# bcsefercik/markerless-robot-camera-calibration

Measured on AMD Instinct MI355X. Metric: point-cloud frames/sec at 200k pts/frame, higher is better.
Workload: dtype f32

## Files before the change

### include/sv_hip.h

```cpp
#ifndef SV_HIP_H
#define SV_HIP_H

#include <stddef.h>
#include <stdint.h>

#ifdef __cplusplus
extern "C" {
#endif

#define SV_OK 0
#define SV_ERR_INVALID (-1)
#define SV_ERR_WORKSPACE (-2)
#define SV_ERR_HIP (-3)
#define SV_ERR_RANGE (-4)
#define SV_ERR_UNSUPPORTED (-5)

#define SV_ACT_NONE 0
#define SV_ACT_RELU 1
#define SV_ACT_LEAKY_RELU 2

#define SV_POOL_MAX 0
#define SV_POOL_AVG 1

#define SV_REDUCE_MEAN 0
// ... 269 lines not shown
                     int max_n, int64_t* out, sv_stream_t stream);
#define SV_PN_MAX_LAYERS 4
int sv_pointnet_sa(const float* xyz, const float* points, const float* new_xyz, const int64_t* group_idx, int B, int N,
                   int D, int S, int nsample, const float* params, const int* widths, int L, float* out,
                   sv_stream_t stream);
#define SV_PN_MAX_SCALES 4
int sv_pointnet_sa_msg(const float* xyz, const float* points, const float* new_xyz, int B, int N, int D, int S, int R,
                       const int* nsamples, const int64_t* const* group_idx, const float* const* params,
                       const int* widths, const int* nlayers, float* out, sv_stream_t stream);

#define SV_GROUP_SSG 0
#define SV_GROUP_MSG 1
int sv_group_rows(const float* xyz, const float* points, const float* new_xyz, const int64_t* idx, int B, int N, int D,
                  int S, int nsample, int order, int ld, float* out, sv_stream_t stream);
size_t sv_index_transpose_workspace_bytes(int B, int64_t M, int N);
int sv_index_transpose(const void* idx, int idx_bytes, int B, int64_t M, int N, void* workspace, size_t workspace_bytes,
                       int32_t* offsets, int32_t* pos, sv_stream_t stream);
int sv_gather_transpose(const int32_t* offsets, const int32_t* pos, const float* w, const float* rows, int64_t ld_rows,
                        int col0, int C, int per_row, int64_t T, float* out, int64_t ld_out, sv_stream_t stream);
int sv_group_max(const float* rows, int64_t ld, int64_t G, int nsample, int C, float* out, int32_t* arg,
                 sv_stream_t stream);
int sv_group_max_backward(const float* dpooled, const int32_t* arg, int64_t G, int nsample, int C, float* drows,
                          sv_stream_t stream);
int sv_three_nn(const float* xyz1, const float* xyz2, int B, int N, int S, int32_t* idx, float* w, sv_stream_t stream);
int sv_three_nn_gather(const float* points2, const int32_t* idx, const float* w, int B, int N, int S, int C, float* out,
                       sv_stream_t stream);

size_t sv_cluster_workspace_bytes(int64_t n);
int sv_single_linkage_roots(const void* xyz, int elem_bytes, int64_t ld, const int32_t* idx, int64_t n, double dist,
                            void* workspace, size_t workspace_bytes, int32_t* root, int32_t* best, sv_stream_t stream);
int sv_select_equal(const void* v, int elem_bytes, int64_t n, int64_t value, const int32_t* value_dev, int64_t* out,
                    int64_t* count, sv_stream_t stream);

#ifdef __cplusplus
}
#endif
#endif
```

### markerless-robot-camera-calibration_amd/_lib.py

```python
import ctypes
import os
import threading
from ctypes import c_char_p, c_double, c_float, c_int, c_int64, c_size_t, c_void_p

import torch

_HERE = os.path.dirname(os.path.abspath(__file__))
ABI_VERSION = 4
LIB_PATH = os.environ.get("SVHIP_LIB") or os.path.join(_HERE, "libsvhip.so")

SV_ACT_NONE, SV_ACT_RELU, SV_ACT_LEAKY_RELU = 0, 1, 2
SV_POOL_MAX, SV_POOL_AVG = 0, 1
SV_REDUCE_MEAN, SV_REDUCE_FIRST = 0, 1
SV_TILE_ROWS = 128
SV_ERR_UNSUPPORTED = -5
SV_PN_MAX_LAYERS = 4
SV_PN_MAX_SCALES = 4
SV_BQ_MAX_RADII = 4
SV_GROUP_SSG, SV_GROUP_MSG = 0, 1
SV_LOSS_POSE, SV_LOSS_SHAPE_MATCH, SV_LOSS_POSE_MATCH, SV_LOSS_KP_POSE_MATCH = 0, 1, 2, 3
SV_AUG_STRIDE, SV_AUG_ELASTIC0, SV_AUG_ELASTIC1 = 40, 0, 7
SV_AUG_E_ON, SV_AUG_E_OFFSET, SV_AUG_E_BX, SV_AUG_E_BY, SV_AUG_E_BZ, SV_AUG_E_GRAN, SV_AUG_E_MAG = range(7)
SV_AUG_NOISE_ON, SV_AUG_NOISE_SIGMA, SV_AUG_NOISE_CLIP, SV_AUG_TRANSFORM_ON, SV_AUG_ROT, SV_AUG_TRANSLATION = 14, 15, 16, 17, 18, 27
SV_AUG_FLIP_SIGN, SV_AUG_GRAVITY_ON, SV_AUG_GRAVITY_ANGLE, SV_AUG_GRAVITY_COS, SV_AUG_GRAVITY_SIN = 30, 31, 32, 33, 34
SV_ORIGIN_NONE, SV_ORIGIN_CENTER, SV_ORIGIN_BASE = 0, 1, 2
SV_COORD_BIAS = 1 << 17
SV_COORD_BITS = 18
SV_MAX_BATCH = 1024
SV_FRAME_MAX_LEVELS, SV_FRAME_MAX_CUTS, SV_FRAME_RECORD = 8, 4, 16
SV_FRAME_K3, SV_FRAME_DOWN, SV_FRAME_UP, SV_FRAME_SPLIT = 1, 2, 4, 8
SV_FIELD_F32, SV_FIELD_F64 = 7, 8
SV_UNPACK_BIGENDIAN, SV_UNPACK_KEEP_NONFINITE = 1, 2
SV_DEPTH_U16, SV_DEPTH_F32 = 4, 7
SV_RGBD_ALIGNED, SV_RGBD_NEAREST, SV_RGBD_BGR = 1, 2, 4
SV_CONV_SEL_PLAN, SV_CONV_SEL_TILE_ORDER, SV_CONV_SEL_VEC_A, SV_CONV_SEL_BUF_OK, SV_CONV_SEL_ACC_INIT, SV_CONV_SEL_W_ALIGNED = (
    1, 2, 4, 8, 16, 32)
SV_FRAME_REC_HASH, SV_FRAME_REC_K3, SV_FRAME_REC_DOWN, SV_FRAME_REC_UP, SV_FRAME_REC_SPLIT = 1, 2, 3, 4, 5


class SvHipError(RuntimeError):
    pass


_P = c_void_p
SIGNATURES = {
    "sv_last_error": (c_char_p, []),
    "sv_abi_version": (c_int, []),
    "sv_voxelize_workspace_bytes": (c_size_t, [c_int64]),
    "sv_voxelize": (c_int, [_P, c_int, c_int64, _P, c_size_t, _P, _P, _P, _P, _P, _P, _P]),
    "sv_voxel_reduce": (c_int, [_P, c_int, _P, _P, c_int64, c_int, _P, _P]),
    "sv_hash_build": (c_int, [_P, c_int64, _P, _P, c_int64, _P]),
    "sv_stride_map_workspace_bytes": (c_size_t, [c_int64]),
    "sv_stride_map": (c_int, [_P, c_int64, c_int, _P, c_size_t, _P, _P, _P, _P, _P, _P]),
    "sv_kernel_map_k3": (c_int, [_P, c_int64, c_int, c_int, _P, _P, c_int64, _P, c_int64, _P, _P]),
    "sv_kernel_map_down": (c_int, [_P, _P, c_int64, c_int, c_int64, _P, c_int64, _P, _P]),
    "sv_kernel_map_up": (c_int, [_P, _P, c_int64, c_int, _P, c_int64, _P, _P]),
    "sv_plan_workspace_bytes": (c_size_t, [c_int64]),
    "sv_plan_build": (c_int, [_P, c_int64, _P, c_int, c_int64, c_int64, _P, c_size_t, _P, _P, _P, _P, c_int64, _P]),
    "sv_conv_fwd": (
        c_int,
        [_P, c_int64, c_int64, c_int, _P, c_int, c_int, _P, _P, _P, _P, c_int64, c_int64, _P, _P, _P, c_int64, c_int,
         c_float, _P, c_int64, _P],
    ),
    "sv_conv_fwd_acc": (
        c_int,
        [_P, c_int64, c_int64, c_int, _P, c_int, c_int, _P, _P, _P, _P, c_int64, c_int64, _P, c_int64, _P, _P, _P, c_int64, c_int,
         c_float, _P, c_int64, _P],
    ),
    "sv_pack_weights_bf16": (c_int, [_P, c_int, c_int, c_int, _P, _P]),
    "sv_conv_fwd_bf16": (
# ... 64 lines not shown
    "sv_pose_match_loss": (c_int, [_P, _P, c_int64, c_int, _P, _P, _P, _P, _P, _P, c_int, _P, c_size_t, _P, _P, _P, _P, _P]),
    "sv_elastic_field_workspace_bytes": (c_size_t, [_P, c_int]),
    "sv_elastic_field": (c_int, [_P, _P, c_int, _P, c_size_t, _P, _P]),
    "sv_augment_points_workspace_bytes": (c_size_t, [c_int64, c_int]),
    "sv_augment_points": (c_int, [_P, c_int, _P, c_int64, c_int, _P, _P, c_int64, _P, _P, c_size_t, _P, _P, _P]),
    "sv_quantise_points": (c_int, [_P, _P, c_int64, c_int, _P, c_int, c_double, _P, _P, _P, _P]),
    "sv_ee_mask": (c_int, [_P, c_int, _P, c_int64, c_int, _P, _P, _P, _P, _P]),
    "sv_key_points": (c_int, [_P, c_int, _P, c_int64, c_int, _P, _P, c_int, c_double, c_int64, _P, _P, _P, _P]),
    "sv_line_topk_workspace_bytes": (c_size_t, [c_int64]),
    "sv_line_topk": (c_int, [_P, c_int, _P, c_int64, c_int, _P, _P, _P, _P, c_int, c_double, _P, c_size_t, _P, _P, _P, _P]),
    "sv_radius_labels": (c_int, [_P, c_int, _P, c_int64, c_int, _P, c_int, c_double, c_int64, _P, _P]),
    "sv_seg_criterion_workspace_bytes": (c_size_t, [c_int64, c_int, c_int]),
    "sv_seg_criterion": (c_int, [_P, c_int64, c_int, c_int64, _P, c_int64, _P, c_int, _P, c_size_t, _P, _P, _P, _P, _P, _P]),
    "sv_segment_topk_workspace_bytes": (c_size_t, [c_int64, c_int, c_int]),
    "sv_segment_topk": (c_int, [_P, c_int64, c_int64, _P, c_int, c_int, _P, c_size_t, _P, _P]),
    "sv_fps": (c_int, [_P, c_int, c_int, c_int, _P, _P, _P]),
    "sv_three_nn_interpolate": (c_int, [_P, _P, _P, c_int, c_int, c_int, c_int, _P, _P]),
    "sv_cluster_workspace_bytes": (c_size_t, [c_int64]),
    "sv_single_linkage_roots": (c_int, [_P, c_int, c_int64, _P, c_int64, c_double, _P, c_size_t, _P, _P, _P]),
    "sv_select_equal": (c_int, [_P, c_int, c_int64, c_int64, _P, _P, _P, _P]),
    "sv_ball_query": (c_int, [_P, _P, c_int, c_int, c_int, c_double, c_int, _P, _P]),
    "sv_fps_segmented": (c_int, [_P, _P, _P, _P, c_int, c_int, _P, _P]),
    "sv_pointnet_sa": (c_int, [_P, _P, _P, _P, c_int, c_int, c_int, c_int, c_int, _P, _P, c_int, _P, _P]),
    "sv_ball_query_multi": (c_int, [_P, _P, c_int, c_int, c_int, c_int, _P, _P, _P, _P]),
    "sv_pointnet_sa_msg": (c_int, [_P, _P, _P, c_int, c_int, c_int, c_int, c_int, _P, _P, _P, _P, _P, _P, _P]),
    "sv_group_rows": (c_int, [_P, _P, _P, _P, c_int, c_int, c_int, c_int, c_int, c_int, c_int, _P, _P]),
    "sv_index_transpose_workspace_bytes": (c_size_t, [c_int, c_int64, c_int]),
    "sv_index_transpose": (c_int, [_P, c_int, c_int, c_int64, c_int, _P, c_size_t, _P, _P, _P]),
    "sv_gather_transpose": (c_int, [_P, _P, _P, _P, c_int64, c_int, c_int, c_int, c_int64, _P, c_int64, _P]),
    "sv_group_max": (c_int, [_P, c_int64, c_int64, c_int, c_int, _P, _P, _P]),
    "sv_group_max_backward": (c_int, [_P, _P, c_int64, c_int, c_int, _P, _P]),
    "sv_three_nn": (c_int, [_P, _P, c_int, c_int, c_int, _P, _P, _P]),
    "sv_three_nn_gather": (c_int, [_P, _P, _P, c_int, c_int, c_int, c_int, _P, _P]),
}

_lib = None


def load():
    global _lib
    if _lib is not None:
        return _lib
    if not os.path.exists(LIB_PATH):
        raise SvHipError(
            f"{LIB_PATH} not found: build it with `python -c 'import __graft_entry__ as g; g.build()'` "
            "(or `make -C markerless-robot-camera-calibration_amd/csrc`). There is no CPU fallback."
        )
    lib = ctypes.CDLL(LIB_PATH)
    lib.sv_abi_version.restype = c_int
    if lib.sv_abi_version() != ABI_VERSION:
        raise SvHipError(f"{LIB_PATH} has C-ABI version {lib.sv_abi_version()}, this package binds version {ABI_VERSION}: "
                         "rebuild it (`python -c 'import __graft_entry__ as g; g.build()'`)")
    for name, (res, args) in SIGNATURES.items():
        fn = getattr(lib, name)
        fn.restype = res
        fn.argtypes = args
    _lib = lib
    return lib


def _check(rc, name):
    if rc != 0:
        msg = _lib.sv_last_error().decode("utf-8", "replace")
        raise SvHipError(f"{name} failed with status {rc}: {msg}")


# ... 62 lines not shown
```

### markerless-robot-camera-calibration_amd/model/robotnet.py

```python
import torch
import torch.nn as nn
import torch.nn.functional as F

from .. import MinkowskiEngine as ME
from .. import nn as svnn
from .._lib import SV_ACT_LEAKY_RELU, SV_ACT_RELU
from ..utils import config
from ._select import pose_backbone


def _linear_fused(linear, x, act=0, slope=0.01):
    w3 = linear.weight.detach().t().contiguous().unsqueeze(0)
    bias = linear.bias.detach() if linear.bias is not None else None
    return svnn.conv_forward(x.contiguous(), w3, None, x.shape[0], None, bias, None, act, slope)


class _PoseHeadMixin:
    def _init_head(self, feat_channels, out_channels, avg_pool):
        cfg = config.Config()
        self.global_pool = ME.MinkowskiGlobalAvgPooling() if avg_pool else ME.MinkowskiGlobalMaxPooling()
        self.final_bn = ME.MinkowskiBatchNorm(out_channels)
        self.output_layer = nn.Sequential(ME.MinkowskiBatchNorm(feat_channels), self.relu)
        self.use_joint_angles = bool(cfg.STRUCTURE.use_joint_angles)
        self.pose_regression_input_size = feat_channels + (9 if self.use_joint_angles else 0)
        self.pose_regression = nn.Sequential(
            nn.Linear(self.pose_regression_input_size, 2048),
            nn.LeakyReLU(),
            nn.Linear(2048, out_channels),
        )

    def _regress(self, feats, joint_angles):
        if self.training:
            return self._regress_train(feats, joint_angles)
        scale, shift = self.output_layer[0].folded()
        feats = feats.new(svnn.affine_act(feats.F, scale, shift, act=SV_ACT_RELU))
        pooled = self.global_pool(feats).features
        if self.use_joint_angles:
            pooled = torch.cat((pooled, joint_angles.to(pooled)), dim=1)
        h = _linear_fused(self.pose_regression[0], pooled, SV_ACT_LEAKY_RELU, self.pose_regression[1].negative_slope)
        out = _linear_fused(self.pose_regression[2], h)
        out[:, 7:] = torch.sigmoid(out[:, 7:])
        if not self.training:
            out[:, 3:7] = F.normalize(out[:, 3:7], p=2, dim=1)
        return out


    def _regress_train(self, feats, joint_angles):
        feats = self.relu(self.output_layer[0](feats))
        pooled = self.global_pool(feats).features
        if self.use_joint_angles:
            pooled = torch.cat((pooled, joint_angles.to(pooled)), dim=1)
        h = svnn.linear_train(self.pose_regression[0], pooled, SV_ACT_LEAKY_RELU, self.pose_regression[1].negative_slope)
        out = svnn.linear_train(self.pose_regression[2], h)
        return torch.cat((out[:, :7], torch.sigmoid(out[:, 7:])), dim=1)


def make_robotnet(backbone=None):
    UNet = pose_backbone(backbone, "ROTATION")

    class RobotNet(UNet, _PoseHeadMixin):
        name = "robotnet"

        def __init__(self, in_channels, out_channels, D=3):
            UNet.__init__(self, in_channels, out_channels, D)
            self.leaky_relu = ME.MinkowskiLeakyReLU(inplace=False)
            self._init_head(self.PLANES[-1] * self.BLOCK.expansion, out_channels, avg_pool=False)

        def forward(self, x):
            joint_angles = None
            if isinstance(x, tuple):
                x, joint_angles = x
            return self._regress(self.forward_except_final(x), joint_angles)

    return RobotNet


def make_robotnet_encode(backbone=None):
    UNet = pose_backbone(backbone, "TRANSLATION")

    class RobotNetEncode(UNet, _PoseHeadMixin):
        name = "robotnet"

        def __init__(self, in_channels, out_channels, D=3):
            UNet.__init__(self, in_channels, out_channels, D)
            cfg = config.Config()
            self.leaky_relu = nn.LeakyReLU()
            self._init_head(self.PLANES[3] * self.BLOCK.expansion, out_channels, avg_pool=True)
            self.quantization_size = cfg()["DATA"].get("quantization_size", 1 / cfg.DATA.scale)
            self.voxelize_position = cfg()["DATA"].get("voxelize_position", False)

        def forward(self, x):
            joint_angles = None
            if isinstance(x, tuple):
                x, joint_angles = x
            out = self.conv0p1s1.forward_fused(x, bn=self.bn0, act=SV_ACT_RELU)
            for i in range(1, 5):
                conv, bn, block = self._down_names(i)
                out = getattr(self, conv).forward_fused(out, bn=getattr(self, bn), act=SV_ACT_RELU)
                out = getattr(self, block)(out)
            out = self._regress(out, joint_angles)
            if not self.training and self.voxelize_position:
                out[:, :3] *= self.quantization_size
            return out

    return RobotNetEncode


RobotNet = make_robotnet()
```

### markerless-robot-camera-calibration_amd/model/robotnet_segmentation.py

```python
import torch.nn as nn

from .. import MinkowskiEngine as ME
from .._lib import SV_ACT_LEAKY_RELU
from ..utils import config
from ._select import pose_backbone, segmentation_backbone

EPS = 1e-6


def _classification_head(UNet, default_classes, class_name):
    class _Head(UNet):
        name = "robotnet"

        def __init__(self, in_channels, out_channels=256, D=3, num_classes=None):
            UNet.__init__(self, in_channels, out_channels, D)
            if num_classes is None:
                num_classes = default_classes()
            self.leaky_relu = ME.MinkowskiLeakyReLU()
            self.regression = nn.Sequential(
                ME.MinkowskiOps.MinkowskiLinear(256, 1024),
                ME.MinkowskiLeakyReLU(),
                ME.MinkowskiOps.MinkowskiLinear(1024, num_classes),
            )
            self.sigm = ME.MinkowskiSigmoid()

        def forward(self, x):
            if isinstance(x, tuple):
                x, _joint_angles = x
            slope = self.leaky_relu.negative_slope
            out = UNet.forward(self, x, final_act=SV_ACT_LEAKY_RELU, final_slope=slope)
            out = self.regression[0].forward_fused(out, act=SV_ACT_LEAKY_RELU,
                                                   slope=self.regression[1].negative_slope)
            return self.regression[2].forward_fused(out)

    _Head.__name__ = _Head.__qualname__ = class_name
    return _Head


def make_robotnet_segmentation(backbone=None):
    return _classification_head(segmentation_backbone(backbone), lambda: config.Config().DATA.classes,
                                "RobotNetSegmentation")


def make_robotnet_vote(backbone=None):
    return _classification_head(pose_backbone(backbone, "ROTATION"),
                                lambda: 2 if config.Config().DATA.data_type == "ee_seg" else 4, "RobotNetVote")


RobotNetSegmentation = make_robotnet_segmentation()
```

### markerless-robot-camera-calibration_amd/nn.py

```python
import math
from ctypes import c_float, c_int, c_int64, c_size_t

import numpy as np
import torch
import torch.nn as nn

from . import _lib, profiling
from ._lib import SV_ACT_LEAKY_RELU, SV_ACT_NONE, SV_ACT_RELU, call, ptr, stream_ptr
from .sparse import SparseTensor, SplitPlan

KERNEL_OFFSET_PERMUTATION = None

import os as _os


def _parse_split_rules(text):
    rules = []
    for part in text.split(";"):
        if part.strip():
            rows, _, cuts = part.partition(":")
            cuts = tuple(int(v) for v in cuts.split(",") if v)
            rules.append((int(rows), cuts[0] if len(cuts) == 1 else cuts))
    return sorted(rules, key=lambda r: -r[0])


SPLIT_RULES = _parse_split_rules(_os.environ.get("MRCC_SPLIT_RULES", "20000:9,18"))
SPLIT_MIN_CHANNELS = int(_os.environ.get("MRCC_SPLIT_MIN_CHANNELS", "128"))


SPLIT_RULES_ONE_FRAME = _parse_split_rules(_os.environ.get("MRCC_SPLIT_RULES_ONE_FRAME", "50000:9,18"))


def split_points_for(rows):
    for min_rows, cuts in SPLIT_RULES:
        if rows >= min_rows:
            return cuts
    return None


def conv_forward(feats, weight3, plan, V_out, scale=None, shift=None, residual=None, act=SV_ACT_NONE, slope=0.01,
                 out=None, weight_bf16=None):
    K, Cin, Cout = weight3.shape
    if feats.shape[1] != Cin:
        raise ValueError(f"input has {feats.shape[1]} channels, kernel expects {Cin}")
    if feats.stride(1) != 1:
        feats = feats.contiguous()
    if out is None:
        out = torch.empty((V_out, Cout), dtype=torch.float32, device=feats.device)
    if isinstance(plan, SplitPlan):
        return _conv_forward_split(feats, weight3, plan, V_out, scale, shift, residual, act, slope, out, weight_bf16)
    return _conv_forward_one(feats, weight3, plan, V_out, scale, shift, residual, act, slope, out, None, wp=weight_bf16)


def pack_weights_bf16(weight3):
    K, Cin, Cout = weight3.shape
    w = weight3.detach().float().contiguous()
    wp = torch.empty(K * Cin * Cout, dtype=torch.bfloat16, device=w.device)
    call("sv_pack_weights_bf16", ptr(w), c_int(K), c_int(Cin), c_int(Cout), ptr(wp), stream_ptr())
    return wp


def _conv_forward_split(feats, weight3, plan, V_out, scale, shift, residual, act, slope, out, weight_bf16=None):
    K, Cin, Cout = weight3.shape
    timer = profiling.TIMER
    t0 = None
    if timer is not None:
        kname = profiling.conv_kernel_config(Cout, plan.Vpad, Cin, plan.parts[-1][1] - plan.parts[-1][0])
        if timer.want(kname):
            t0 = timer.start()
    if weight_bf16 is None and not weight3.is_contiguous():
        weight3 = weight3.contiguous()
    acc = None
    for i, (k0, k1, sub) in enumerate(plan.parts):
        w = weight3[k0:k1]
        wp = weight_bf16[k0 * Cin * Cout:k1 * Cin * Cout] if weight_bf16 is not None else None
        if i == len(plan.parts) - 1:
            _conv_forward_one(feats, w, sub, V_out, scale, shift, residual, act, slope, out, acc, timed=False, wp=wp)
        else:
            nxt = torch.empty((V_out, Cout), dtype=torch.float32, device=feats.device)
            _conv_forward_one(feats, w, sub, V_out, None, None, None, SV_ACT_NONE, slope, nxt, acc, timed=False, wp=wp)
            acc = nxt
    if t0 is not None:
        timer.stop(t0, _lib.conv_last_instance()[0], K, Cin, Cout, V_out, plan.pairs_device(), level=plan.out_stride,
                   passes=len(plan.parts))
# ... 613 lines not shown
```

### markerless-robot-camera-calibration_amd/profiling.py

```python
import math

import torch

from . import _lib

TIMER = None
INSTANCE_LOG = None
TRAIN_LOG = None


def conv_kernel_config(Cout, Vpad, Cin, K=1):
    flags = _lib.SV_CONV_SEL_BUF_OK | _lib.SV_CONV_SEL_W_ALIGNED
    if K > 1:
        flags |= _lib.SV_CONV_SEL_PLAN | _lib.SV_CONV_SEL_TILE_ORDER
    if Cin % 4 == 0:
        flags |= _lib.SV_CONV_SEL_VEC_A
    return _lib.conv_instance(K, Cin, Cout, Vpad, flags).partition("|")[0]


class KernelTimer:
    def __init__(self, capacity=0):
        self.records = []
        self.enabled = True
        self.only = None
        self._pool = [torch.cuda.Event(enable_timing=True) for _ in range(capacity)]
        self._next = 0
        self._first_of_frame = False

    def _event(self):
        if self._next < len(self._pool):
            e = self._pool[self._next]
            self._next += 1
            return e
        return torch.cuda.Event(enable_timing=True)

    def want(self, kernel):
        return self.enabled and (self.only is None or kernel in self.only)

    def start(self):
        e = self._event()
        e.record()
        return e

    def stop(self, start_evt, kernel, K, Cin, Cout, V_out, pairs_dev, level=None, passes=1):
        e = self._event()
        e.record()
        self.records.append((kernel, K, Cin, Cout, V_out, pairs_dev, start_evt, e, self._first_of_frame, level, passes))
        self._first_of_frame = False

    def frame_boundary(self):
        self._first_of_frame = True

    def clear(self):
        self.records = []

    @staticmethod
    def layer_key(kernel, K, Cin, Cout, V_out, level=None):
        where = f"s{level}" if level is not None else f"~2^{int(round(math.log2(max(V_out, 1))))}"
        return (kernel, K, Cin, Cout, where)

    def summarize(self, by_layer=False):
        out = {}
        for kernel, K, Cin, Cout, V_out, pairs_dev, s, e, first, level, passes in self.records:
            if first:
                continue
            P = int(pairs_dev.item()) if pairs_dev is not None else V_out
            ms = s.elapsed_time(e)
            key = self.layer_key(kernel, K, Cin, Cout, V_out, level) if by_layer else kernel
            d = out.setdefault(key, {"launches": 0, "ms": 0.0, "flops": 0.0, "bytes": 0.0, "rows": 0.0, "kernel_launches": 0})
            d["rows"] += V_out
            d["launches"] += 1
            d["kernel_launches"] += passes
            d["ms"] += ms
            d["flops"] += 2.0 * P * Cin * Cout
            d["bytes"] += P * (4.0 * Cin + 8) + 4.0 * V_out * Cout + 4.0 * K * Cin * Cout
        return out


def pass_gflop(fn):
    global TIMER
# ... 8 lines not shown
```

Measured before the change: 74.65.

## Compile eval network into an op program executed by one native call

Adds a net executor that compiles the RobotNet/segmentation forward into a flat array of op records (conv, bf16 conv, column copy, affine, pool, event wait/record). A single C entry point then launches them all in sequence. Activations live in one preallocated arena with precomputed offsets, and concatenations become column copies into that arena. The aim is to remove per-layer Python dispatch, tensor allocation and ctypes overhead in inference. It adds a large compile and layout-check layer and falls back to layer-by-layer execution for unrecognised modules.

```diff
diff --git a/include/sv_hip.h b/include/sv_hip.h
--- a/include/sv_hip.h
+++ b/include/sv_hip.h
@@ -325,6 +325,41 @@
 int sv_select_equal(const void* v, int elem_bytes, int64_t n, int64_t value, const int32_t* value_dev, int64_t* out,
                     int64_t* count, sv_stream_t stream);
 
+#define SV_NET_NOP 0
+#define SV_NET_CONV 1
+#define SV_NET_CONV_BF16 2
+#define SV_NET_COPY_COLS 3
+#define SV_NET_AFFINE 4
+#define SV_NET_POOL 5
+#define SV_NET_WAIT_EVENT 6
+#define SV_NET_RECORD_EVENT 7
+#define SV_NET_NAME_BYTES 128
+typedef struct sv_net_op {
+  int32_t kind, Cin, K, Cout, act;
+  float slope;
+  int32_t B, mode;
+  const void* in;
+  int64_t V_in, in_ld;
+  const void* W;
+  const int32_t* perm;
+  const int32_t* nbr_s;
+  const uint32_t* submask;
+  const int32_t* tile_order;
+  int64_t V_out, Vpad;
+  const float* acc_init;
+  int64_t acc_ld;
+  const float* scale;
+  const float* shift;
+  const float* residual;
+  int64_t res_ld;
+  void* out;
+  int64_t out_ld;
+  void* event;
+  char* name_host;
+} sv_net_op;
+int sv_net_op_layout(int64_t* out_host, int capacity);
+int sv_net_forward(const sv_net_op* ops, int n, int* failed_index, sv_stream_t stream);
+
 #ifdef __cplusplus
 }
 #endif
diff --git a/markerless-robot-camera-calibration_amd/_lib.py b/markerless-robot-camera-calibration_amd/_lib.py
--- a/markerless-robot-camera-calibration_amd/_lib.py
+++ b/markerless-robot-camera-calibration_amd/_lib.py
@@ -36,6 +36,9 @@
 SV_CONV_SEL_PLAN, SV_CONV_SEL_TILE_ORDER, SV_CONV_SEL_VEC_A, SV_CONV_SEL_BUF_OK, SV_CONV_SEL_ACC_INIT, SV_CONV_SEL_W_ALIGNED = (
     1, 2, 4, 8, 16, 32)
 SV_FRAME_REC_HASH, SV_FRAME_REC_K3, SV_FRAME_REC_DOWN, SV_FRAME_REC_UP, SV_FRAME_REC_SPLIT = 1, 2, 3, 4, 5
+(SV_NET_NOP, SV_NET_CONV, SV_NET_CONV_BF16, SV_NET_COPY_COLS, SV_NET_AFFINE, SV_NET_POOL, SV_NET_WAIT_EVENT,
+ SV_NET_RECORD_EVENT) = range(8)
+SV_NET_NAME_BYTES = 128
 
 
 class SvHipError(RuntimeError):
@@ -166,6 +169,8 @@
     "sv_group_max_backward": (c_int, [_P, _P, c_int64, c_int, c_int, _P, _P]),
     "sv_three_nn": (c_int, [_P, _P, c_int, c_int, c_int, _P, _P, _P]),
     "sv_three_nn_gather": (c_int, [_P, _P, _P, c_int, c_int, c_int, c_int, _P, _P]),
+    "sv_net_op_layout": (c_int, [_P, c_int]),
+    "sv_net_forward": (c_int, [_P, c_int, _P, _P]),
 }
 
 _lib = None
diff --git a/markerless-robot-camera-calibration_amd/csrc/sv_net.hip b/markerless-robot-camera-calibration_amd/csrc/sv_net.hip
--- /dev/null
+++ b/markerless-robot-camera-calibration_amd/csrc/sv_net.hip
@@ -0,0 +1,110 @@
+#include <stddef.h>
+#include <string.h>
+
+#include "sv_common.h"
+
+namespace sv {
+
+template <typename T>
+__global__ __launch_bounds__(256) void copy_cols_kernel(const T* __restrict__ in, int64_t in_ld, T* __restrict__ out, int64_t out_ld,
+                                                        int64_t rows, int cols) {
+  const int64_t total = rows * (int64_t)cols;
+  for (int64_t i = (int64_t)blockIdx.x * blockDim.x + threadIdx.x; i < total; i += (int64_t)gridDim.x * blockDim.x) {
+    const int64_t r = i / cols;
+    const int c = (int)(i - r * cols);
+    out[r * out_ld + c] = in[r * in_ld + c];
+  }
+}
+
+static int copy_cols(const sv_net_op& op, hipStream_t stream) {
+  const float* in = (const float*)op.in;
+  float* out = (float*)op.out;
+  const int cols = op.Cout;
+  const int64_t rows = op.V_out;
+  SV_CHECK_ARG(cols > 0 && rows >= 0 && op.in_ld >= cols && op.out_ld >= cols, "bad column count / row strides");
+  if (rows == 0) return SV_OK;
+  SV_CHECK_ARG(in && out, "null pointer");
+  const bool vec = cols % 4 == 0 && op.in_ld % 4 == 0 && op.out_ld % 4 == 0 && (((uintptr_t)in | (uintptr_t)out) & 15) == 0;
+  const int64_t total = rows * (int64_t)(vec ? cols / 4 : cols);
+  int64_t blocks = (total + 255) / 256;
+  if (blocks > 65536) blocks = 65536;
+  if (vec)
+    copy_cols_kernel<float4><<<dim3((unsigned)blocks), dim3(256), 0, stream>>>((const float4*)in, op.in_ld / 4, (float4*)out, op.out_ld / 4,
+                                                                              rows, cols / 4);
+  else
+    copy_cols_kernel<float><<<dim3((unsigned)blocks), dim3(256), 0, stream>>>(in, op.in_ld, out, op.out_ld, rows, cols);
+  SV_LAUNCH_CHECK();
+  return SV_OK;
+}
+
+static int run_op(const sv_net_op& op, hipStream_t stream) {
+  sv_stream_t st = (sv_stream_t)stream;
+  switch (op.kind) {
+    case SV_NET_NOP:
+      return SV_OK;
+    case SV_NET_CONV:
+      return sv_conv_fwd_acc((const float*)op.in, op.V_in, op.in_ld, op.Cin, (const float*)op.W, op.K, op.Cout, op.perm, op.nbr_s,
+                             op.submask, op.tile_order, op.V_out, op.Vpad, op.acc_init, op.acc_ld, op.scale, op.shift, op.residual,
+                             op.res_ld, op.act, op.slope, (float*)op.out, op.out_ld, st);
+    case SV_NET_CONV_BF16:
+      return sv_conv_fwd_bf16((const float*)op.in, op.V_in, op.in_ld, op.Cin, (const uint16_t*)op.W, op.K, op.Cout, op.perm, op.nbr_s,
+                              op.submask, op.tile_order, op.V_out, op.Vpad, op.acc_init, op.acc_ld, op.scale, op.shift, op.residual,
+                              op.res_ld, op.act, op.slope, (float*)op.out, op.out_ld, st);
+    case SV_NET_COPY_COLS:
+      return copy_cols(op, stream);
+    case SV_NET_AFFINE:
+      return sv_affine_act((const float*)op.in, op.in_ld, op.Cout, op.V_out, op.scale, op.shift, op.residual, op.res_ld, op.act,
+                           op.slope, (float*)op.out, op.out_ld, st);
+    case SV_NET_POOL:
+      return sv_global_pool((const float*)op.in, op.in_ld, op.Cin, op.perm, op.B, op.mode, (float*)op.out, st);
+    case SV_NET_WAIT_EVENT:
+      if (op.event) SV_HIP(hipStreamWaitEvent(stream, (hipEvent_t)op.event, 0));
+      return SV_OK;
+    case SV_NET_RECORD_EVENT:
+      if (op.event) SV_HIP(hipEventRecord((hipEvent_t)op.event, stream));
+      return SV_OK;
+    default:
+      set_error("sv_net_forward: unknown op kind %d", op.kind);
+      return SV_ERR_INVALID;
+  }
+}
+
+}
+
+extern "C" int sv_net_op_layout(int64_t* out_host, int capacity) {
+#define SV_NET_FIELD(f) offsetof(sv_net_op, f)
+  static const size_t offs[] = {
+      SV_NET_FIELD(kind),    SV_NET_FIELD(Cin),     SV_NET_FIELD(K),        SV_NET_FIELD(Cout),       SV_NET_FIELD(act),
+      SV_NET_FIELD(slope),   SV_NET_FIELD(B),       SV_NET_FIELD(mode),     SV_NET_FIELD(in),         SV_NET_FIELD(V_in),
+      SV_NET_FIELD(in_ld),   SV_NET_FIELD(W),       SV_NET_FIELD(perm),     SV_NET_FIELD(nbr_s),      SV_NET_FIELD(submask),
+      SV_NET_FIELD(tile_order), SV_NET_FIELD(V_out), SV_NET_FIELD(Vpad),    SV_NET_FIELD(acc_init),   SV_NET_FIELD(acc_ld),
+      SV_NET_FIELD(scale),   SV_NET_FIELD(shift),   SV_NET_FIELD(residual), SV_NET_FIELD(res_ld),     SV_NET_FIELD(out),
+      SV_NET_FIELD(out_ld),  SV_NET_FIELD(event),   SV_NET_FIELD(name_host)};
+#undef SV_NET_FIELD
+  const int nf = (int)(sizeof(offs) / sizeof(offs[0]));
+  SV_CHECK_ARG(out_host && capacity >= 2 + nf, "out_host holds 2 + the field count entries");
+  out_host[0] = (int64_t)sizeof(sv_net_op);
+  out_host[1] = nf;
+  for (int i = 0; i < nf; ++i) out_host[2 + i] = (int64_t)offs[i];
+  return SV_OK;
+}
+
+extern "C" int sv_net_forward(const sv_net_op* ops, int n, int* failed_index, sv_stream_t stream_) {
+  if (failed_index) *failed_index = -1;
+  SV_CHECK_ARG(n >= 0 && (n == 0 || ops), "null op list");
+  hipStream_t stream = (hipStream_t)stream_;
+  for (int i = 0; i < n; ++i) {
+    const sv_net_op& op = ops[i];
+    const int rc = sv::run_op(op, stream);
+    if (rc != SV_OK) {
+      if (failed_index) *failed_index = i;
+      return rc;
+    }
+    if (op.name_host) {
+      const bool conv = op.kind == SV_NET_CONV || op.kind == SV_NET_CONV_BF16;
+      strncpy(op.name_host, conv ? sv_conv_last_instance() : "", SV_NET_NAME_BYTES - 1);
+      op.name_host[SV_NET_NAME_BYTES - 1] = '\0';
+    }
+  }
+  return SV_OK;
+}
diff --git a/markerless-robot-camera-calibration_amd/model/robotnet.py b/markerless-robot-camera-calibration_amd/model/robotnet.py
--- a/markerless-robot-camera-calibration_amd/model/robotnet.py
+++ b/markerless-robot-camera-calibration_amd/model/robotnet.py
@@ -3,6 +3,7 @@
 import torch.nn.functional as F
 
 from .. import MinkowskiEngine as ME
+from .. import net_program
 from .. import nn as svnn
 from .._lib import SV_ACT_LEAKY_RELU, SV_ACT_RELU
 from ..utils import config
@@ -34,7 +35,9 @@
             return self._regress_train(feats, joint_angles)
         scale, shift = self.output_layer[0].folded()
         feats = feats.new(svnn.affine_act(feats.F, scale, shift, act=SV_ACT_RELU))
-        pooled = self.global_pool(feats).features
+        return self._regress_pooled(self.global_pool(feats).features, joint_angles)
+
+    def _regress_pooled(self, pooled, joint_angles):
         if self.use_joint_angles:
             pooled = torch.cat((pooled, joint_angles.to(pooled)), dim=1)
         h = _linear_fused(self.pose_regression[0], pooled, SV_ACT_LEAKY_RELU, self.pose_regression[1].negative_slope)
@@ -70,6 +73,9 @@
             joint_angles = None
             if isinstance(x, tuple):
                 x, joint_angles = x
+            pooled = net_program.forward(self, x, "unet_pool")
+            if pooled is not None:
+                return self._regress_pooled(pooled, joint_angles)
             return self._regress(self.forward_except_final(x), joint_angles)
 
     return RobotNet
@@ -93,6 +99,12 @@
             joint_angles = None
             if isinstance(x, tuple):
                 x, joint_angles = x
+            pooled = net_program.forward(self, x, "encoder_pool")
+            if pooled is not None:
+                out = self._regress_pooled(pooled, joint_angles)
+                if self.voxelize_position:
+                    out[:, :3] *= self.quantization_size
+                return out
             out = self.conv0p1s1.forward_fused(x, bn=self.bn0, act=SV_ACT_RELU)
             for i in range(1, 5):
                 conv, bn, block = self._down_names(i)
diff --git a/markerless-robot-camera-calibration_amd/model/robotnet_segmentation.py b/markerless-robot-camera-calibration_amd/model/robotnet_segmentation.py
--- a/markerless-robot-camera-calibration_amd/model/robotnet_segmentation.py
+++ b/markerless-robot-camera-calibration_amd/model/robotnet_segmentation.py
@@ -1,6 +1,7 @@
 import torch.nn as nn
 
 from .. import MinkowskiEngine as ME
+from .. import net_program
 from .._lib import SV_ACT_LEAKY_RELU
 from ..utils import config
 from ._select import pose_backbone, segmentation_backbone
@@ -27,6 +28,9 @@
         def forward(self, x):
             if isinstance(x, tuple):
                 x, _joint_angles = x
+            out = net_program.forward(self, x, "classify")
+            if out is not None:
+                return out
             slope = self.leaky_relu.negative_slope
             out = UNet.forward(self, x, final_act=SV_ACT_LEAKY_RELU, final_slope=slope)
             out = self.regression[0].forward_fused(out, act=SV_ACT_LEAKY_RELU,
diff --git a/markerless-robot-camera-calibration_amd/net_program.py b/markerless-robot-camera-calibration_amd/net_program.py
--- /dev/null
+++ b/markerless-robot-camera-calibration_amd/net_program.py
@@ -0,0 +1,581 @@
+import ctypes
+import logging
+import os
+import threading
+import weakref
+from ctypes import c_int, c_int64, c_void_p
+
+import numpy as np
+import torch
+
+from . import _lib, profiling
+from ._lib import SV_ACT_LEAKY_RELU, SV_ACT_NONE, SV_ACT_RELU
+from .sparse import BUF_LIMIT, SparseTensor
+
+log = logging.getLogger(__name__)
+
+OP_FIELDS = [("kind", "<i4"), ("Cin", "<i4"), ("K", "<i4"), ("Cout", "<i4"), ("act", "<i4"), ("slope", "<f4"), ("B", "<i4"),
+             ("mode", "<i4"), ("in", "<u8"), ("V_in", "<i8"), ("in_ld", "<i8"), ("W", "<u8"), ("perm", "<u8"), ("nbr_s", "<u8"),
+             ("submask", "<u8"), ("tile_order", "<u8"), ("V_out", "<i8"), ("Vpad", "<i8"), ("acc_init", "<u8"), ("acc_ld", "<i8"),
+             ("scale", "<u8"), ("shift", "<u8"), ("residual", "<u8"), ("res_ld", "<i8"), ("out", "<u8"), ("out_ld", "<i8"),
+             ("event", "<u8"), ("name_host", "<u8")]
+OP_DTYPE = np.dtype(OP_FIELDS, align=True)
+
+ROW_ALIGN = 64
+BATCH = "B"
+
+
+def enabled():
+    return os.environ.get("MRCC_NET_EXECUTOR", "1") != "0"
+
+
+def library_layout():
+    out = (c_int64 * 64)()
+    _lib.call("sv_net_op_layout", out, c_int(64))
+    return int(out[0]), [int(out[2 + i]) for i in range(int(out[1]))]
+
+
+_layout_ok = False
+
+
+def _check_layout():
+    global _layout_ok
+    if not _layout_ok:
+        size, offs = library_layout()
+        mine = [OP_DTYPE.fields[name][1] for name, _ in OP_FIELDS]
+        if size != OP_DTYPE.itemsize or offs != mine:
+            raise _lib.SvHipError(f"sv_net_op: the library lays the record out as {size} bytes {offs}, this binding as "
+                                  f"{OP_DTYPE.itemsize} bytes {mine}: rebuild libsvhip.so")
+        _layout_ok = True
+
+
+class Unrecognised(Exception):
+    """the compiler does not know this module's forward: it runs layer by layer"""
+
+
+class Buf:
+    __slots__ = ("id", "level", "cols")
+
+    def __init__(self, id, level, cols):
+        self.id, self.level, self.cols = id, level, cols
+
+
+class Op:
+
+    def __init__(self, kind, **kw):
+        self.kind = kind
+        self.__dict__.update(kw)
+
+
+def _conv_geometry(layer, level):
+    from . import nn as svnn
+
+    if isinstance(layer, svnn.MinkowskiLinear):
+        return 1, layer.linear.in_features, layer.linear.out_features, None, level, False
+    if not isinstance(layer, svnn._ConvBase):
+        raise Unrecognised(f"{type(layer).__name__} is not a conv / linear layer")
+    ks, st, Cin, Cout = layer.kernel_size, layer.stride, layer.in_channels, layer.out_channels
+    if not layer.transposed:
+        if ks == 1 and st == 1:
+            return 1, Cin, Cout, None, level, False
+        if ks == 3 and st == 1:
+            split_ok = layer.dilation == 1 and Cin >= svnn.SPLIT_MIN_CHANNELS and Cout >= svnn.SPLIT_MIN_CHANNELS
+            return 27, Cin, Cout, ("k3", level, layer.dilation), level, split_ok
+        if ks == 2 and st == 2:
+            return 8, Cin, Cout, ("down", level), level * 2, False
+    elif ks == 2 and st == 2 and level >= 2:
+        return 8, Cin, Cout, ("up", level), level // 2, False
+    raise Unrecognised(f"kernel_size={ks} stride={st} transposed={layer.transposed}")
+
+
+class Program:
+
+    def __init__(self, module, what):
+        self.what = what
+        self.ops = []
+        self.bufs = [Buf(0, 1, module.conv0p1s1.in_channels)]
+        self.lock = threading.Lock()
+        self._templates = {}
+        self._compile(module, what)
+        self.layers = [op.layer for op in self.ops if op.kind == "conv"]
+        self.modules = self.layers + [op.bn for op in self.ops if getattr(op, "bn", None) is not None]
+        self.split_levels = sorted({op.plan[1] for op in self.ops if op.kind == "conv" and op.split_ok})
+        self.signature = self._signature()
+
+    def _tensors(self):
+        from . import nn as svnn
+
+        for m in self.modules:
+            if isinstance(m, svnn.MinkowskiBatchNorm):
+                yield from (m.bn.weight, m.bn.bias, m.bn.running_mean, m.bn.running_var)
+            elif isinstance(m, svnn.MinkowskiLinear):
+                yield from (m.linear.weight, m.linear.bias)
+            else:
+                yield from (m.kernel, m.bias)
+
+    def _signature(self):
+        from .nn import _tensor_versions
+
+        return tuple(m.compute_precision for m in self.layers), _tensor_versions(*self._tensors())
+
+    def in_eval(self):
+        return not any(m.training for m in self.modules)
+
+    def _new(self, level, cols):
+        b = Buf(len(self.bufs), level, cols)
+        self.bufs.append(b)
+        return b
+
+    def _conv(self, layer, src, bn=None, residual=None, act=SV_ACT_NONE, slope=0.01, cat_with=None):
+        K, Cin, Cout, plan, out_level, split_ok = _conv_geometry(layer, src.level)
+        if src.cols != Cin:
+            raise ValueError(f"input has {src.cols} channels, kernel expects {Cin}")
+        if bn is not None and getattr(layer, "bias", None) is not None:
+            raise Unrecognised("conv bias followed by a fused BatchNorm")
+        if residual is not None and (residual.level != out_level or residual.cols != Cout):
+            raise Unrecognised("residual on another map")
+        if cat_with is not None and cat_with.level != out_level:
+            raise ValueError("ME.cat needs tensors on the same coordinate map")
+        dst = self._new(out_level, Cout + (cat_with.cols if cat_with is not None else 0))
+        self.ops.append(Op("conv", layer=layer, bn=bn, K=K, Cin=Cin, Cout=Cout, plan=plan, split_ok=split_ok, src=src, dst=dst,
+                           dst_col=0, residual=residual, act=act, slope=slope))
+        if cat_with is not None:
+            self.ops.append(Op("copy", src=cat_with, dst=dst, dst_col=Cout, cols=cat_with.cols))
+        return dst
+
+    def _block(self, b, x):
+        from .nn import BasicBlock, Bottleneck
+
+        ds = None
+        if b.downsample is not None:
+            if len(b.downsample) != 2:
+                raise Unrecognised("downsample is not (conv, BN)")
+            ds = (b.downsample[0], b.downsample[1])
+        if type(b) is BasicBlock:
+            out = self._conv(b.conv1, x, bn=b.norm1, act=SV_ACT_RELU)
+            residual = self._conv(ds[0], x, bn=ds[1]) if ds else x
+            return self._conv(b.conv2, out, bn=b.norm2, residual=residual, act=SV_ACT_RELU)
+        if type(b) is Bottleneck:
+            out = self._conv(b.conv1, x, bn=b.norm1, act=SV_ACT_RELU)
+            out = self._conv(b.conv2, out, bn=b.norm2, act=SV_ACT_RELU)
+            residual = self._conv(ds[0], x, bn=ds[1]) if ds else x
+            return self._conv(b.conv3, out, bn=b.norm3, residual=residual, act=SV_ACT_RELU)
+        raise Unrecognised(f"block {type(b).__name__}")
+
+    def _stack(self, blocks, x):
+        for b in blocks:
+            x = self._block(b, x)
+        return x
+
+    def _encode(self, m, x, stages):
+        out = self._conv(m.conv0p1s1, x, bn=m.bn0, act=SV_ACT_RELU)
+        skips = [out]
+        for i in range(1, stages + 1):
+            conv, bn, block = m._down_names(i)
+            out = self._conv(getattr(m, conv), out, bn=getattr(m, bn), act=SV_ACT_RELU)
+            out = self._stack(getattr(m, block), out)
+            skips.append(out)
+        return skips.pop(), skips
+
+    def _except_final(self, m, x):
+        n = m.N_LEVELS
+        out, skips = self._encode(m, x, n)
+        for j in range(n, 2 * n):
+            conv, bn, block = m._up_names(j)
+            if j == 2 * n - 1:
+                self.ops.append(Op("hook", name="level0_begin"))
+            out = self._conv(getattr(m, conv), out, bn=getattr(m, bn), act=SV_ACT_RELU, cat_with=skips.pop())
+            out = self._stack(getattr(m, block), out)
+            if j == 2 * n - 1:
+                self.ops.append(Op("hook", name="level0_end"))
+        return out
+
+    def _compile(self, m, what):
+        from .model.backbone.aliveunet import AliveUNetBase
+        from .model.backbone.minkunet import MinkUNetBase
+
+        cls = type(m)
+        if not isinstance(m, MinkUNetBase) or cls.encode is not MinkUNetBase.encode \
+                or cls.forward_except_final is not MinkUNetBase.forward_except_final:
+            raise Unrecognised(f"{cls.__name__} does not run MinkUNetBase's forward")
+        x = self.bufs[0]
+        if what == "classify":
+            if isinstance(m, AliveUNetBase):
+                raise Unrecognised(f"{cls.__name__}: no `final` in this backbone's forward")
+            slope = m.leaky_relu.negative_slope
+            out = self._except_final(m, x)
+            out = self._conv(m.final, out, act=SV_ACT_LEAKY_RELU, slope=slope)
+            out = self._conv(m.regression[0], out, act=SV_ACT_LEAKY_RELU, slope=m.regression[1].negative_slope)
+            out = self._conv(m.regression[2], out)
+        elif what in ("unet_pool", "encoder_pool"):
+            out = self._except_final(m, x) if what == "unet_pool" else self._encode(m, x, 4)[0]
+            bn = m.output_layer[0]
+            if bn.bn.num_features != out.cols:
+                raise ValueError(f"output_layer normalises {bn.bn.num_features} channels, the body gives {out.cols}")
+            act = self._new(out.level, out.cols)
+            self.ops.append(Op("affine", bn=bn, src=out, dst=act, act=SV_ACT_RELU))
+            from .nn import MinkowskiGlobalAvgPooling
+
+            mode = _lib.SV_POOL_AVG if isinstance(m.global_pool, MinkowskiGlobalAvgPooling) else _lib.SV_POOL_MAX
+            out = self._new(BATCH, out.cols)
+            self.ops.append(Op("pool", src=act, dst=out, mode=mode))
+        else:
+            raise ValueError(what)
+        self.out = out
+
+    def template(self, cuts_key):
+        t = self._templates.get(cuts_key)
+        if t is None:
+            with self.lock:
+                t = self._templates.get(cuts_key)
+                if t is None:
+                    t = self._templates[cuts_key] = Template(self, dict(zip(self.split_levels, cuts_key)))
+        return t
+
+    def run(self, x):
+        sig = self._signature()
+        if sig != self.signature:
+            with self.lock:
+                self._templates = {}
+                self.signature = sig
+        cm = x.coordinate_manager
+        key = tuple(cm.split_cuts_for(cm.stride_map(l).V) for l in self.split_levels)
+        return self.template(key).run(x)
+
+
+def _bounds(cuts):
+    return (0,) + ((cuts,) if isinstance(cuts, int) else tuple(cuts)) + (27,)
+
+
+def assign_columns(bufs, intervals):
+    col0, peak, placed = {}, {}, {}
+    for i in sorted(bufs, key=lambda i: (intervals[i][0], i)):
+        b = bufs[i]
+        first, last = intervals[i]
+        busy = sorted((col0[j], col0[j] + bufs[j].cols) for j in placed.get(b.level, ())
+                      if intervals[j][1] >= first and intervals[j][0] <= last)
+        c = 0
+        for lo, hi in busy:
+            if c + b.cols <= lo:
+                break
+            c = max(c, hi)
+        col0[i] = c
+        placed.setdefault(b.level, []).append(i)
+        peak[b.level] = max(peak.get(b.level, 0), c + b.cols)
+    return col0, peak
+
+
+class Template:
+
+    def __init__(self, prog, cuts):
+        self.prog = prog
+        self.cuts = cuts
+        self.keep = []
+        bufs = {b.id: b for b in prog.bufs}
+        recs = []
+        self.boundaries = []
+        self.layers = []
+        self.wait = -1
+        slots = {}
+
+        def slot(key):
+            return slots.setdefault(key, len(slots)) if key is not None else -1
+
+        def new_buf(level, cols):
+            b = Buf(len(bufs), level, cols)
+            bufs[b.id] = b
+            return b
+
+        for op in prog.ops:
+            if op.kind == "hook":
+                self.boundaries.append((len(recs), op.name))
+            elif op.kind == "copy":
+                recs.append(dict(kind=_lib.SV_NET_COPY_COLS, Cout=op.cols, _in=(op.src, 0), _out=(op.dst, op.dst_col),
+                                 _rows=op.dst.level))
+            elif op.kind == "affine":
+                scale, shift = op.bn.folded()
+                self.keep += [scale, shift]
+                recs.append(dict(kind=_lib.SV_NET_AFFINE, Cout=op.src.cols, act=op.act, slope=0.01, scale=scale.data_ptr(),
+                                 shift=shift.data_ptr(), _in=(op.src, 0), _out=(op.dst, 0), _rows=op.src.level))
+            elif op.kind == "pool":
+                recs.append(dict(kind=_lib.SV_NET_POOL, Cin=op.src.cols, mode=op.mode, _in=(op.src, 0), _out=(op.dst, 0),
+                                 _rows=op.src.level, _pool=True))
+            else:
+                self._expand_conv(op, recs, slot, new_buf)
+        self.n = n = len(recs)
+
+        first, last = {}, {}
+        for r, rec in enumerate(recs):
+            for key in ("_in", "_res", "_acc"):
+                if rec.get(key) is not None:
+                    last[rec[key][0].id] = r
+            if rec.get("_out") is not None:
+                first.setdefault(rec["_out"][0].id, r)
+        last[prog.out.id] = n
+        arena_bufs = {i: b for i, b in bufs.items() if i != 0}
+        self.intervals = {i: (first[i], max(last.get(i, first[i]), first[i])) for i in arena_bufs}
+        self.col0, peak = assign_columns(arena_bufs, self.intervals)
+        self.bufs = bufs
+        self.levels = sorted({b.level for b in bufs.values()}, key=lambda l: (l == BATCH, l if l != BATCH else 0))
+        lvl = {l: i for i, l in enumerate(self.levels)}
+        self.level_peak = np.array([peak.get(l, 0) for l in self.levels], np.int64)
+        nb = len(bufs)
+        self.buf_level = np.array([lvl[bufs[i].level] for i in range(nb)], np.int64)
+        self.buf_col0 = np.array([self.col0.get(i, 0) for i in range(nb)], np.int64)
+
+        base = np.zeros(n, OP_DTYPE)
+        ix = {k: np.full(n, -1, np.int64) for k in ("in_buf", "out_buf", "res_buf", "acc_buf", "lvl_in", "lvl_out", "slot")}
+        col = {k: np.zeros(n, np.int64) for k in ("in", "out", "res")}
+        for r, rec in enumerate(recs):
+            for f, v in rec.items():
+                if not f.startswith("_"):
+                    base[f][r] = v
+            for key, bname, ld in (("_in", "in", "in_ld"), ("_out", "out", "out_ld"), ("_res", "res", "res_ld"),
+                                   ("_acc", "acc", "acc_ld")):
+                if rec.get(key) is not None:
+                    b, c = rec[key]
+                    ix[bname + "_buf"][r] = b.id
+                    if bname != "acc":
+                        col[bname][r] = c
+                    base[ld][r] = b.cols
+            if rec.get("_in") is not None:
+                ix["lvl_in"][r] = lvl[rec["_in"][0].level]
+            if rec.get("_rows") is not None:
+                ix["lvl_out"][r] = lvl[rec["_rows"]]
+            ix["slot"][r] = rec.get("_slot", -1)
+        self.base, self.ix, self.col = base, ix, col
+        self.has = {k: np.nonzero(ix[k] >= 0)[0] for k in ix}
+        self.dense = np.nonzero((ix["slot"] < 0) & ((base["kind"] == _lib.SV_NET_CONV) | (base["kind"] == _lib.SV_NET_CONV_BF16)))[0]
+        self.ext_in = np.nonzero(ix["in_buf"] == 0)[0]
+        self.ext_res = np.nonzero(ix["res_buf"] == 0)[0]
+        self.pools = [r for r, rec in enumerate(recs) if rec.get("_pool")]
+        self.is_conv = (base["kind"] == _lib.SV_NET_CONV) | (base["kind"] == _lib.SV_NET_CONV_BF16)
+        self.convs = np.nonzero(self.is_conv)[0]
+        self.slot_keys = sorted(slots, key=slots.get)
+        self.out_level = lvl[prog.out.level]
+        self.planned = np.nonzero(self.is_conv & (ix["slot"] >= 0))[0]
+        self.out_row_bytes = 4 * np.maximum(np.maximum(base["out_ld"], base["res_ld"]), base["acc_ld"])[self.planned]
+
+    def _expand_conv(self, op, recs, slot, new_buf):
+        layer, Cin, Cout = op.layer, op.Cin, op.Cout
+        scale = shift = None
+        if op.bn is not None:
+            scale, shift = op.bn.folded()
+        else:
+            bias = layer.linear.bias if hasattr(layer, "linear") else layer.bias
+            if bias is not None:
+                shift = bias.detach().reshape(-1)
+        wp = layer._weight_bf16()
+        if wp is None:
+            w = layer.weight3().detach()
+            if not w.is_contiguous():
+                w = w.contiguous()
+            kind, esize = _lib.SV_NET_CONV, 4
+        else:
+            w, kind, esize = wp, _lib.SV_NET_CONV_BF16, 2
+        self.keep += [w, scale, shift]
+        ptr = lambda t: t.data_ptr() if t is not None else 0
+        cuts = self.cuts.get(op.plan[1]) if op.split_ok else None
+        common = dict(kind=kind, Cin=Cin, Cout=Cout, slope=op.slope, _in=(op.src, 0), _rows=op.dst.level)
+        epilogue = dict(act=op.act, scale=ptr(scale), shift=ptr(shift), _res=(op.residual, 0) if op.residual is not None else None,
+                        _out=(op.dst, op.dst_col))
+        first = len(recs)
+        if cuts is None:
+            recs.append(dict(common, K=op.K, W=w.data_ptr(), _slot=slot(op.plan), **epilogue))
+        else:
+            if self.wait < 0:
+                self.wait = len(recs)
+                recs.append(dict(kind=_lib.SV_NET_WAIT_EVENT))
+                first += 1
+            b = _bounds(cuts)
+            acc = None
+            for i, (k0, k1) in enumerate(zip(b[:-1], b[1:])):
+                rec = dict(common, K=k1 - k0, W=w.data_ptr() + k0 * Cin * Cout * esize,
+                           _slot=slot(("k3split", op.plan[1], cuts, i)), _acc=(acc, 0) if acc is not None else None)
+                if i == len(b) - 2:
+                    rec.update(epilogue)
+                else:
+                    acc = new_buf(op.dst.level, Cout)
+                    rec.update(act=SV_ACT_NONE, _out=(acc, 0))
+                recs.append(rec)
+        whole = slot(op.plan) if cuts is None else slot(("k3", op.plan[1], 1))
+        self.layers.append((first, len(recs) - 1, op.K, Cin, Cout, whole))
+
+    def _plan(self, cm, key):
+        if key[0] == "k3":
+            return cm.plan_k3(key[1], key[2])
+        if key[0] == "down":
+            return cm.plan_down(key[1])
+        if key[0] == "up":
+            return cm.plan_up(key[1])
+        return cm.plan_k3_split(key[1], key[2]).parts[key[3]][2]
+
+    def run(self, x):
+        _check_layout()
+        cm = x.coordinate_manager
+        F = x.F
+        if F.stride(1) != 1:
+            F = F.contiguous()
+        ix, has = self.ix, self.has
+        if BATCH in self.levels and cm.num_batches is None:
+            m = cm.stride_map(1)
+            cm.num_batches = int(m.coords[:, 0].max().item()) + 1 if m.V else 1
+        Vs = np.array([cm.num_batches if l == BATCH else cm.stride_map(l).V for l in self.levels], np.int64)
+        if F.shape[0] != Vs[0] or F.shape[1] != self.bufs[0].cols:
+            raise ValueError(f"input is {tuple(F.shape)}, the network expects ({Vs[0]}, {self.bufs[0].cols})")
+        if Vs.min() < 1:
+            return None
+        event = 0
+        if self.wait >= 0 and cm.split_ready is not None:
+            if all(("k3split", k[1], k[2]) in cm.plans for k in self.slot_keys if k[0] == "k3split"):
+                keep_event = cm.split_ready
+                event = keep_event.cuda_event
+            else:
+                torch.cuda.current_stream().wait_event(cm.split_ready)
+            cm.split_ready = None
+        plans = [self._plan(cm, k) for k in self.slot_keys]
+        V_in, V_out = Vs[ix["lvl_in"]], Vs[ix["lvl_out"]]
+        if len(self.planned) and ((V_in[self.planned] * 4 * self.base["in_ld"][self.planned]).max() >= BUF_LIMIT or
+                                  (V_out[self.planned] * self.out_row_bytes).max() >= BUF_LIMIT):
+            if event:
+                torch.cuda.current_stream().wait_event(keep_event)
+            return None
+        rows = (Vs + ROW_ALIGN - 1) // ROW_ALIGN * ROW_ALIGN
+        share = self.level_peak * rows * 4
+        total = int(share.sum())
+        grain = (32 << 20) if total > (64 << 20) else (2 << 20)
+        arena = torch.empty((total + grain - 1) // grain * grain, dtype=torch.uint8, device=F.device)
+        start = np.cumsum(share) - share
+        buf_ptr = arena.data_ptr() + start[self.buf_level] + self.buf_col0 * rows[self.buf_level] * 4
+        buf_ptr[0] = F.data_ptr()
+
+        recs = self.base.copy()
+        for name, field in (("in", "in"), ("out", "out"), ("res", "residual")):
+            h = has[name + "_buf"]
+            recs[field][h] = buf_ptr[ix[name + "_buf"][h]] + 4 * self.col[name][h]
+        h = has["acc_buf"]
+        recs["acc_init"][h] = buf_ptr[ix["acc_buf"][h]]
+        recs["in_ld"][self.ext_in] = F.stride(0)
+        recs["res_ld"][self.ext_res] = F.stride(0)
+        h = has["lvl_in"]
+        recs["V_in"][h] = V_in[h]
+        h = has["lvl_out"]
+        recs["V_out"][h] = V_out[h]
+        recs["Vpad"][self.dense] = (np.maximum(V_out[self.dense], 1) + _lib.SV_TILE_ROWS - 1) // _lib.SV_TILE_ROWS * _lib.SV_TILE_ROWS
+        if plans:
+            h = has["slot"]
+            s = ix["slot"][h]
+            for field in ("perm", "nbr_s", "submask", "tile_order"):
+                recs[field][h] = np.array([getattr(p, field).data_ptr() for p in plans], np.uint64)[s]
+            recs["Vpad"][h] = np.array([p.Vpad for p in plans], np.int64)[s]
+        for r in self.pools:
+            B = int(cm.num_batches)
+            recs["perm"][r] = cm.batch_offsets(self.levels[ix["lvl_in"][r]], B).data_ptr()
+            recs["B"][r] = B
+        if event:
+            recs["event"][self.wait] = event
+
+        timer, ilog = profiling.TIMER, profiling.INSTANCE_LOG
+        boundaries = self.boundaries if cm.phase_hook is not None else []
+        if timer is None and ilog is None:
+            self._walk(recs, boundaries, cm.phase_hook)
+        else:
+            self._walk_observed(recs, boundaries, cm, plans, timer, ilog)
+
+        lo = int(buf_ptr[self.prog.out.id]) - arena.data_ptr()
+        Vo, Co = int(Vs[self.out_level]), self.prog.out.cols
+        out = arena[lo: lo + 4 * Vo * Co].view(torch.float32).view(Vo, Co)
+        if self.prog.out.level == BATCH:
+            return out
+        return SparseTensor(out, coordinate_manager=cm, tensor_stride=self.prog.out.level, _internal=True)
+
+    def _walk(self, recs, boundaries, hook):
+        lib = _lib.load()
+        failed = c_int(-1)
+        stride = OP_DTYPE.itemsize
+        base = recs.ctypes.data
+        at = 0
+        for end, name in list(boundaries) + [(len(recs), None)]:
+            if end > at:
+                rc = lib.sv_net_forward(c_void_p(base + at * stride), c_int(end - at), ctypes.byref(failed), _lib.stream_ptr())
+                if rc != 0:
+                    msg = lib.sv_last_error().decode("utf-8", "replace")
+                    raise _lib.SvHipError(f"sv_net_forward failed with status {rc} at op {at + failed.value}: {msg}")
+            at = end
+            if name is not None:
+                hook(name)
+
+    def _walk_observed(self, recs, boundaries, cm, plans, timer, ilog):
+        n = len(recs)
+        names = np.zeros((n, _lib.SV_NET_NAME_BYTES), np.uint8)
+        recs["name_host"][self.convs] = names.ctypes.data + _lib.SV_NET_NAME_BYTES * self.convs
+        before, after, timed = {}, {}, []
+        if timer is not None:
+            st = torch.cuda.current_stream()
+            for first, last, K, Cin, Cout, whole in self.layers:
+                kname = profiling.conv_kernel_config(Cout, int(recs["Vpad"][last]), Cin, int(recs["K"][last]))
+                if timer.want(kname):
+                    e0, e1 = timer._event(), timer._event()
+                    e0.record(st)
+                    e1.record(st)
+                    before[first], after[last] = e0.cuda_event, e1.cuda_event
+                    timed.append((first, last, K, Cin, Cout, whole, e0, e1))
+        order, pos = [], {}
+        for r in range(n):
+            pos[r] = len(order)
+            if r in before:
+                order.append(("event", before[r]))
+            order.append(("op", r))
+            if r in after:
+                order.append(("event", after[r]))
+        pos[n] = len(order)
+        full = np.zeros(len(order), OP_DTYPE)
+        for i, (what, v) in enumerate(order):
+            if what == "op":
+                full[i] = recs[v]
+            else:
+                full["kind"][i] = _lib.SV_NET_RECORD_EVENT
+                full["event"][i] = v
+        self._walk(full, [(pos[r], name) for r, name in boundaries], cm.phase_hook)
+        name_of = lambda r: bytes(names[r]).split(b"\0", 1)[0].decode()
+        if ilog is not None:
+            for r in self.convs:
+                ilog.append((*_lib._parse_instance(name_of(r)), int(recs["K"][r]), int(recs["Cin"][r]), int(recs["Cout"][r]),
+                             int(recs["V_out"][r])))
+        for first, last, K, Cin, Cout, whole, e0, e1 in timed:
+            pairs, level = (plans[whole].pairs_device(), plans[whole].out_stride) if whole >= 0 else (None, None)
+            timer.file(e0, e1, _lib._parse_instance(name_of(last))[0], K, Cin, Cout, int(recs["V_out"][last]), pairs,
+                       level=level, passes=last - first + 1)
+
+
+_programs = weakref.WeakKeyDictionary()
+_programs_lock = threading.Lock()
+
+
+def program_for(module, what):
+    per = _programs.get(module)
+    if per is None or what not in per:
+        with _programs_lock:
+            per = _programs.setdefault(module, {})
+            if what not in per:
+                try:
+                    per[what] = Program(module, what)
+                except Unrecognised as e:
+                    log.warning("%s runs layer by layer: the net executor does not recognise it (%s)", type(module).__name__, e)
+                    per[what] = None
+    return per[what]
+
+
+def forward(module, x, what):
+    if module.training or not enabled() or not isinstance(x, SparseTensor) or x.tensor_stride != 1:
+        return None
+    if x.F.requires_grad and torch.is_grad_enabled():
+        return None
+    from . import nn as svnn
+
+    if svnn.conv_forward is not svnn.LAYER_CONV_FORWARD:
+        return None
+    prog = program_for(module, what)
+    if prog is None or not prog.in_eval():
+        return None
+    return prog.run(x)
diff --git a/markerless-robot-camera-calibration_amd/nn.py b/markerless-robot-camera-calibration_amd/nn.py
--- a/markerless-robot-camera-calibration_amd/nn.py
+++ b/markerless-robot-camera-calibration_amd/nn.py
@@ -50,6 +50,9 @@
     if isinstance(plan, SplitPlan):
         return _conv_forward_split(feats, weight3, plan, V_out, scale, shift, residual, act, slope, out, weight_bf16)
     return _conv_forward_one(feats, weight3, plan, V_out, scale, shift, residual, act, slope, out, None, wp=weight_bf16)
+
+
+LAYER_CONV_FORWARD = conv_forward
 
 
 def pack_weights_bf16(weight3):
diff --git a/markerless-robot-camera-calibration_amd/profiling.py b/markerless-robot-camera-calibration_amd/profiling.py
--- a/markerless-robot-camera-calibration_amd/profiling.py
+++ b/markerless-robot-camera-calibration_amd/profiling.py
@@ -45,7 +45,10 @@
     def stop(self, start_evt, kernel, K, Cin, Cout, V_out, pairs_dev, level=None, passes=1):
         e = self._event()
         e.record()
-        self.records.append((kernel, K, Cin, Cout, V_out, pairs_dev, start_evt, e, self._first_of_frame, level, passes))
+        self.file(start_evt, e, kernel, K, Cin, Cout, V_out, pairs_dev, level, passes)
+
+    def file(self, start_evt, stop_evt, kernel, K, Cin, Cout, V_out, pairs_dev, level=None, passes=1):
+        self.records.append((kernel, K, Cin, Cout, V_out, pairs_dev, start_evt, stop_evt, self._first_of_frame, level, passes))
         self._first_of_frame = False
 
     def frame_boundary(self):
```

New measurement: 74.75, median of 6. About the same (+0.1%).
